# mazpie/genrl

Measured on AMD Instinct MI355X. Metric: world-model+imag update steps/sec (B32xL32x64x64x3), higher is better.
Workload: dtype f32 (storage, accumulation, every non-GEMM kernel and the fp32-MFMA GEMMs; the forward / dgrad / weight-gradient products of the imagination rollout, of the Dense+LN+SiLU chains from 192 rows up and of the encoder / decoder convolutions take fp32 operands pre-split into two fp16 planes of the scaled

## Files before the change

### genrl_amd/csrc/gemm_planes.hip

```cpp
#include "common.h"
#include "genrl_hip.h"
#include <type_traits>

typedef __bf16 bf16x8_t __attribute__((ext_vector_type(8)));
typedef _Float16 f16x8_t __attribute__((ext_vector_type(8)));
typedef unsigned u32x4 __attribute__((ext_vector_type(4)));

namespace {

struct PlaneSeg {
  const u16* a; long a_ld, a_plane;
  const u16* b; long b_ld, b_plane;
  int k;
  const float* a_inv; const float* b_inv;
};

struct SampleEpi {
  const float* q;
  long ldq;
  float* sample; long lds;
  u16* sp; long sld, splane; float* sinv;
  float a;
};

// ... 465 lines not shown
      if (ln.rstd) ln.rstd[row] = rs;
      if (ln.yinv) ln.yinv[row] = u_inv;
    }
    if (row < M) {
#pragma unroll
      for (int gq = 0; gq < 4; ++gq) {
        const int col = n0 + wn * 32 + 8 * gq + 4 * h32;
        const f32x4 g = ldsf4(LN_G + 4 * col), b = ldsf4(LN_B + 4 * col);
        float y[4];
#pragma unroll
        for (int v = 0; v < 4; ++v) {
          const float z = (o[4 * gq + v] - mu) * rs * g[v] + b[v];
          y[v] = ln.act ? siluf_(z) : z;
        }
        if (ln.y) *reinterpret_cast<float4*>(ln.y + (long)row * ln.ldy + col) = make_float4(y[0], y[1], y[2], y[3]);
        if (ln.yp) {
          h2_u32x2 hh, ll;
          unsigned a, bq;
          h2_split2(y[0] * u_sc, y[1] * u_sc, a, bq); hh[0] = a; ll[0] = bq;
          h2_split2(y[2] * u_sc, y[3] * u_sc, a, bq); hh[1] = a; ll[1] = bq;
          u16* qd = ln.yp + (long)row * ln.yld + col;
          *reinterpret_cast<h2_u32x2*>(qd) = hh;
          *reinterpret_cast<h2_u32x2*>(qd + ln.yplane) = ll;
        }
      }
    }
    return;
  }
  const float* ainv = ainv_l;
  const float* binv = binv_l;
  auto epi_f = [&](int idx) __attribute__((always_inline)) -> float {
    return *reinterpret_cast<const __attribute__((address_space(3))) float*>((uintptr_t)(lds0 + EPI_AT + 4 * idx));
  };
  auto epi_f4 = [&](int idx) __attribute__((always_inline)) -> float4 {
    typedef float f32x4_ __attribute__((ext_vector_type(4)));
    const f32x4_ t = *reinterpret_cast<const __attribute__((address_space(3))) f32x4_*>((uintptr_t)(lds0 + EPI_AT + 4 * idx));
    return make_float4(t[0], t[1], t[2], t[3]);
  };
  const bool vec_c = ((ldc & 3) == 0) && (((reinterpret_cast<uintptr_t>(C) | reinterpret_cast<uintptr_t>(bias)) & 15) == 0);
#pragma unroll
  for (int i = 0; i < TM; ++i) {
    const int row = m0 + (wm * TM + i) * 32 + l32;
    if (row >= M) continue;
    const float ra = ainv ? (FMT == 1 ? epi_f((wm * TM + i) * 32 + l32) : ainv[row]) : 1.f;
    float lg[16];
#pragma unroll
    for (int j = 0; j < TN; ++j)
#pragma unroll
      for (int gq = 0; gq < 4; ++gq) {
        const int col = n0 + (wn * TN + j) * 32 + 8 * gq + 4 * h32;
        if (col >= N) continue;
        float o[4];
        float cbv[4] = {1.f, 1.f, 1.f, 1.f}, bsv[4] = {0.f, 0.f, 0.f, 0.f};
        if constexpr (FMT == 1) {
          const int ci = (wn * TN + j) * 32 + 8 * gq + 4 * h32;
          if (binv) { const float4 t = epi_f4(BM + ci); cbv[0] = t.x; cbv[1] = t.y; cbv[2] = t.z; cbv[3] = t.w; }
          if (bias) { const float4 t = epi_f4(BM + BN + ci); bsv[0] = t.x; bsv[1] = t.y; bsv[2] = t.z; bsv[3] = t.w; }
        }
#pragma unroll
        for (int v = 0; v < 4; ++v) {
          if constexpr (FMT == 0) {
            float x = acc[0][i][j][4 * gq + v];
#pragma unroll
            for (int c = 1; c < NACC; ++c) x += acc[c][i][j][4 * gq + v];
            o[v] = x;
          } else {
            const float lo = NACC == 3 ? acc[0][i][j][4 * gq + v] + acc[2][i][j][4 * gq + v] : acc[0][i][j][4 * gq + v];
            const float x = lo * (1.f / 2048.f) + acc[1][i][j][4 * gq + v];
            o[v] = x * ra * cbv[v];
          }
        }
        float* c = C + (long)row * ldc + col;
        if (vec_c && col + 3 < N) {
          if constexpr (FMT == 1) {
            o[0] += bsv[0]; o[1] += bsv[1]; o[2] += bsv[2]; o[3] += bsv[3];
          } else if (bias) {
            const float4 bv = *reinterpret_cast<const float4*>(bias + col);
            o[0] += bv.x; o[1] += bv.y; o[2] += bv.z; o[3] += bv.w;
          }
          if (accumulate) {
            const float4 cv = *reinterpret_cast<const float4*>(c);
            o[0] += cv.x; o[1] += cv.y; o[2] += cv.z; o[3] += cv.w;
          }
          *reinterpret_cast<float4*>(c) = make_float4(o[0], o[1], o[2], o[3]);
          if constexpr (TM * TN == 1 && FMT == 1) {
#pragma unroll
            for (int v = 0; v < 4; ++v) lg[4 * gq + v] = o[v];
          }
        } else {
#pragma unroll
          for (int v = 0; v < 4; ++v)
            if (col + v < N) {
              float val = o[v] + (FMT == 1 ? bsv[v] : (bias ? bias[col + v] : 0.f));
              if (accumulate) val += c[v];
              c[v] = val;
            }
        }
      }
    if constexpr (TM * TN == 1 && FMT == 1) {
      if (smp.q) {
        const int c0 = n0 + wn * 32;
        float m = lg[0];
#pragma unroll
        for (int v = 1; v < 16; ++v) m = fmaxf(m, lg[v]);
        m = fmaxf(m, __shfl_xor(m, 32, 64));
        float e[16], z = 0.f;
#pragma unroll
        for (int v = 0; v < 16; ++v) { e[v] = expf(lg[v] - m); z += e[v]; }
        z += __shfl_xor(z, 32, 64);
        float ssum = 0.f;
#pragma unroll
        for (int v = 0; v < 16; ++v) { e[v] = smp.a * (e[v] / z) + (1.0f - smp.a) / 32.0f; ssum += e[v]; }
        ssum += __shfl_xor(ssum, 32, 64);
        float best = -INFINITY; int bi = 0;
#pragma unroll
        for (int gq = 0; gq < 4; ++gq) {
          const int cl = 8 * gq + 4 * h32;
          const float4 qv = *reinterpret_cast<const float4*>(smp.q + (long)row * smp.ldq + c0 + cl);
          const float qq[4] = {qv.x, qv.y, qv.z, qv.w};
#pragma unroll
          for (int v = 0; v < 4; ++v) {
            const float sc = (e[4 * gq + v] / ssum) / qq[v];
            if (sc > best) { best = sc; bi = cl + v; }
          }
        }
        {
          const float ob = __shfl_xor(best, 32, 64);
          const int oi = __shfl_xor(bi, 32, 64);
          if (ob > best || (ob == best && oi < bi)) { best = ob; bi = oi; }
        }
#pragma unroll
        for (int gq = 0; gq < 4; ++gq) {
          const int cl = 8 * gq + 4 * h32;
          float4 oh;
          oh.x = (cl + 0 == bi) ? 1.f : 0.f; oh.y = (cl + 1 == bi) ? 1.f : 0.f;
          oh.z = (cl + 2 == bi) ? 1.f : 0.f; oh.w = (cl + 3 == bi) ? 1.f : 0.f;
          *reinterpret_cast<float4*>(smp.sample + (long)row * smp.lds + c0 + cl) = oh;
          if (smp.sp) {
            h2_u32x2 hh;
            hh[0] = (oh.x != 0.f ? 0x7400u : 0u) | (oh.y != 0.f ? 0x74000000u : 0u);
            hh[1] = (oh.z != 0.f ? 0x7400u : 0u) | (oh.w != 0.f ? 0x74000000u : 0u);
            u16* qd = smp.sp + (long)row * smp.sld + c0 + cl;
            *reinterpret_cast<h2_u32x2*>(qd) = hh;
            *reinterpret_cast<h2_u32x2*>(qd + smp.splane) = h2_u32x2{0u, 0u};
          }
        }
        if (smp.sinv && c0 == 0 && h32 == 0) smp.sinv[row] = 1.f / 16384.f;
      }
    }
  }
  wait_vm<0>();
}

constexpr int HL_KBH = 2, HL_KBL = 2;
template <bool CONV>
__global__ __launch_bounds__(256, 1) void gemm_planes_hl_kernel(PlaneSeg s0, float* __restrict__ C, long ldc, const float* __restrict__ bias,
                                                                int M, int N, int accumulate, int tiles_m, int tiles_n, int xcd_m,
                                                                ConvGather cg) {
  constexpr int BM = 128, BN = 128, ROWB = 128, HALF = (BM + BN) * ROWB, NS = 4, NP = 8, KS = 4;
  constexpr int EPI = 4 * (BM + 2 * BN), EPI_AT = NS * HALF;
  __shared__ __attribute__((aligned(1024))) unsigned char lds[EPI_AT + EPI];
  int tile_m, tile_n;
  {
    int bid = blockIdx.x;
    const int ntiles = tiles_m * tiles_n;
    const int x = bid % 8, i = bid / 8;
    const int order = xcd_m >> 8;
    xcd_m &= 255;
    if (xcd_m > 0) {
      const int sub_m = tiles_m / xcd_m, sub_n = tiles_n / (8 / xcd_m);
      const int xm = x / (8 / xcd_m), xn = x % (8 / xcd_m);
      int im = i / sub_n, in = i % sub_n;
      if (order == 1 && sub_m % 8 == 0 && sub_n % 4 == 0) {
        const int nb_n = sub_n / 4, blk = i / 32, j = i % 32;
        const int rb = blk / nb_n, cbq = blk % nb_n, cb = (rb & 1) ? nb_n - 1 - cbq : cbq;
        im = rb * 8 + j / 4; in = cb * 4 + j % 4;
      } else if (order == 2) {
        im = i % sub_m; in = i / sub_m;
      }
      tile_m = xm * sub_m + im;
      tile_n = xn * sub_n + in;
    } else {
      const int q = ntiles / 8, r = ntiles % 8;
      bid = (x < r ? x * (q + 1) : r * (q + 1) + (x - r) * q) + i;
      tile_m = bid / tiles_n;
      tile_n = bid % tiles_n;
    }
  }
  const int m0 = tile_m * BM, n0 = tile_n * BN;
  const int lane = threadIdx.x & 63;
  const int wave = __builtin_amdgcn_readfirstlane(threadIdx.x >> 6);
  const int wm = wave >> 1, wn = wave & 1;
  const unsigned lds0 = (unsigned)(uintptr_t)lds;
  const bool isB = wave >= 2;
  const int r_in = lane >> 3, slot = lane & 7;
  const char* gbase = reinterpret_cast<const char*>(isB ? s0.b : s0.a);
  const long plane_bytes = (isB ? s0.b_plane : s0.a_plane) * 2;
  unsigned voff[NP];
  unsigned koff[2] = {0u, 0u};
  int kch[2] = {0, 0}, kkw[2] = {0, 0}, kkk[2] = {0, 0};
  if (CONV && !isB) {
    const long ld = s0.a_ld;
#pragma unroll
    for (int i = 0; i < NP; ++i) {
      const int row = ((wave & 1) * NP + i) * 8 + r_in;
      const int m = min(m0 + row, M - 1);
      const int n_img = m / (cg.Ho * cg.Wo), rem = m - n_img * (cg.Ho * cg.Wo);
      const int oy = rem / cg.Wo, ox = rem - oy * cg.Wo;
      voff[i] = (unsigned)((((long)(n_img * cg.H + cg.s * oy) * cg.W + cg.s * ox) * ld) * 2);
    }
#pragma unroll
    for (int par = 0; par < 2; ++par) {
      const int f = (4 * par + (r_in >> 1)) & 7;
      const int kk = 8 * (slot ^ f);
      const int tap = kk / cg.C, ch = kk - tap * cg.C, kh = tap / cg.k, kw = tap - kh * cg.k;
      kkk[par] = kk; kch[par] = ch; kkw[par] = kw;
      koff[par] = (unsigned)((((long)kh * cg.W + kw) * ld + ch) * 2);
    }
  } else {
    const long ld = isB ? s0.b_ld : s0.a_ld;
    const int rows_total = isB ? N : M, r0 = isB ? n0 : m0;
#pragma unroll
    for (int i = 0; i < NP; ++i) {
      const int row = ((wave & 1) * NP + i) * 8 + r_in;
      const int f = (row >> 1) & 7;
      voff[i] = (unsigned)(((long)min(r0 + row, rows_total - 1) * ld) * 2 + ((slot ^ f) << 4));
    }
  }
  const unsigned piece0 = lds0 + (isB ? BM * ROWB : 0) + (wave & 1) * NP * 1024;
  const int l32 = lane & 31, h32 = lane >> 5;
  const int f_rd = (l32 >> 1) & 7;
  unsigned a_s[KS], b_s[KS];
#pragma unroll
  for (int s = 0; s < KS; ++s) {
    const unsigned xo = (unsigned)(((2 * s + h32) ^ f_rd) << 4);
    a_s[s] = lds0 + (wm * 64 + l32) * ROWB + xo;
    b_s[s] = lds0 + BM * ROWB + (wn * 64 + l32) * ROWB + xo;
  }
  f32x16 acc[2][2][2];
#pragma unroll
  for (int c = 0; c < 2; ++c)
#pragma unroll
    for (int i = 0; i < 2; ++i)
#pragma unroll
      for (int j = 0; j < 2; ++j)
#pragma unroll
        for (int r = 0; r < 16; ++r) acc[c][i][j][r] = 0.f;
  u32x4 Hf[2][KS][4], Lf[KS][4];
  auto ldfrag = [&](unsigned addr) __attribute__((always_inline)) -> u32x4 {
    return *reinterpret_cast<const __attribute__((address_space(3))) u32x4*>((uintptr_t)addr);
  };
  auto read_one = [&](u32x4 (&dst)[KS][4], int r, int buf) __attribute__((always_inline)) {
    const int s = r >> 2, blk = r & 3;
    dst[s][blk] = blk < 2 ? ldfrag(a_s[s] + blk * 32 * ROWB + buf * HALF) : ldfrag(b_s[s] + (blk - 2) * 32 * ROWB + buf * HALF);
  };
  auto mma = [&](f32x16& c, const u32x4& bfr, const u32x4& afr) __attribute__((always_inline)) {
    c = __builtin_amdgcn_mfma_f32_32x32x16_f16(__builtin_bit_cast(f16x8_t, bfr), __builtin_bit_cast(f16x8_t, afr), c, 0, 0, 0);
  };
  {
    const float* src = wave == 0 ? s0.a_inv : (wave == 1 ? s0.b_inv : (wave == 2 ? bias : nullptr));
    const int base = wave == 0 ? m0 : n0, lim = (wave == 0 ? M : N) - 1;
    const unsigned dst = lds0 + EPI_AT + (wave == 0 ? 0 : (wave == 1 ? 4 * BM : 4 * (BM + BN)));
    if (src) {
#pragma unroll
      for (int j = 0; j < 2; ++j)
        __builtin_amdgcn_global_load_lds((const __attribute__((address_space(1))) void*)(src + min(base + 64 * j + lane, lim)),
                                         (__attribute__((address_space(3))) void*)(uintptr_t)(dst + 256 * j), 4, 0, 0);
    }
  }
  const int nu = 2 * (s0.k / 64);
  int issued = 0;
  auto next_half = [&]() __attribute__((always_inline)) {
    if (issued > 0 && issued < nu) {
      if (issued & 1) gbase += plane_bytes;
      else {
        gbase += 128 - plane_bytes;
        if constexpr (CONV) {
          if (!isB) {
            gbase -= 128;
            const unsigned ld2 = (unsigned)(s0.a_ld * 2);
#pragma unroll
            for (int par = 0; par < 2; ++par) {
              if (kkk[par] + 64 + 8 <= cg.K) {
                kkk[par] += 64;
                int ch = kch[par] + 64, kw = kkw[par];
                unsigned off = koff[par] + 128u;
#pragma unroll
                for (int rep = 0; rep < 2; ++rep)
                  if (ch >= cg.C) {
                    ch -= cg.C; off -= (unsigned)(cg.C * 2);
                    ++kw; off += ld2;
                    if (kw == cg.k) { kw = 0; off += (unsigned)(cg.W - cg.k) * ld2; }
                  }
                kch[par] = ch; kkw[par] = kw; koff[par] = off;
              }
            }
          }
        }
      }
    }
    ++issued;
  };
  auto issue_one = [&](int buf, int i) __attribute__((always_inline)) {
    if constexpr (CONV) {
      if (!isB) { glds16(gbase + (size_t)(voff[i] + koff[i & 1]), piece0 + buf * HALF + i * 1024); return; }
    }
    glds16(gbase + (size_t)voff[i], piece0 + buf * HALF + i * 1024);
  };
#pragma unroll
  for (int st = 0; st < NS; ++st) {
    next_half();
#pragma unroll
    for (int i = 0; i < NP; ++i) issue_one(st, i);
  }
  next_half();
  wait_vm<(NS - 1) * NP>();
  __builtin_amdgcn_s_barrier();
#pragma unroll
  for (int r = 0; r < 16; ++r) read_one(Hf[0], r, 0);

  int u = 0;
  auto half_iter = [&](auto UC) __attribute__((always_inline)) {
    constexpr int U = decltype(UC)::value;
    constexpr bool LPH = (U & 1) != 0;
    constexpr int HS = U >> 1;
    constexpr int NM = LPH ? 32 : 16, KB = LPH ? HL_KBL : HL_KBH, NSIDE = 16 + NP;
    constexpr int PER = (NSIDE + (NM - KB) - 1) / (NM - KB);
    static_assert((NSIDE + PER - 1) / PER <= NM - KB, "not enough MFMAs to carry the side operations");
    auto mfma_one = [&](int m) __attribute__((always_inline)) {
      if constexpr (!LPH) {
        const int s = m >> 2, i = (m >> 1) & 1, j = m & 1;
        mma(acc[1][i][j], Hf[HS][s][2 + j], Hf[HS][s][i]);
      } else {
        const int s = m >> 3, t = (m >> 2) & 1, i = (m >> 1) & 1, j = m & 1;
        if (t == 0) mma(acc[0][i][j], Hf[HS][s][2 + j], Lf[s][i]);
        else mma(acc[0][i][j], Lf[s][2 + j], Hf[HS][s][i]);
      }
    };
#pragma unroll
    for (int m = 0; m < KB; ++m) mfma_one(m);
    __builtin_amdgcn_sched_barrier(0);
    wait_vm<(NS - 2) * NP>();
    asm volatile("s_waitcnt lgkmcnt(0)" ::: "memory");
    __builtin_amdgcn_s_barrier();
    __builtin_amdgcn_sched_barrier(0);
#pragma unroll
    for (int m = KB; m < NM; ++m) {
      mfma_one(m);
#pragma unroll
      for (int o = (m - KB) * PER; o < (m - KB + 1) * PER; ++o) {
        if (o >= NSIDE) continue;
        if (o % 3 == 2) {
          issue_one(U, o / 3);
        } else {
          const int r = o - o / 3;
          if constexpr (LPH) read_one(Hf[1 - HS], r, (U + 1) % NS);
          else read_one(Lf, r, (U + 1) % NS);
        }
      }
      __builtin_amdgcn_sched_barrier(0);
    }
    next_half();
    ++u;
  };
  while (u + 4 <= nu) {
    half_iter(std::integral_constant<int, 0>{});
    half_iter(std::integral_constant<int, 1>{});
    half_iter(std::integral_constant<int, 2>{});
    half_iter(std::integral_constant<int, 3>{});
  }
  if (u < nu) {
    half_iter(std::integral_constant<int, 0>{});
    half_iter(std::integral_constant<int, 1>{});
  }

  auto epi_f = [&](int idx) __attribute__((always_inline)) -> float {
    return *reinterpret_cast<const __attribute__((address_space(3))) float*>((uintptr_t)(lds0 + EPI_AT + 4 * idx));
  };
  auto epi_f4 = [&](int idx) __attribute__((always_inline)) -> float4 {
    typedef float f32x4_ __attribute__((ext_vector_type(4)));
    const f32x4_ t = *reinterpret_cast<const __attribute__((address_space(3))) f32x4_*>((uintptr_t)(lds0 + EPI_AT + 4 * idx));
    return make_float4(t[0], t[1], t[2], t[3]);
  };
  const bool vec_c = ((ldc & 3) == 0) && (((reinterpret_cast<uintptr_t>(C) | reinterpret_cast<uintptr_t>(bias)) & 15) == 0);
  const bool shuffle = CONV && cg.sCo > 0;
#pragma unroll
  for (int i = 0; i < 2; ++i) {
    const int row = m0 + (wm * 2 + i) * 32 + l32;
    if (row >= M) continue;
    const float ra = s0.a_inv ? epi_f((wm * 2 + i) * 32 + l32) : 1.f;
    int s_py = 0, s_px = 0; long s_img = 0;
    if (shuffle) {
      const int per = cg.Ho * cg.Wo, n_img = row / per, rem = row - n_img * per;
      s_py = rem / cg.Wo; s_px = rem - s_py * cg.Wo;
      s_img = (long)n_img * cg.sHo;
    }
#pragma unroll
    for (int j = 0; j < 2; ++j)
#pragma unroll
      for (int gq = 0; gq < 4; ++gq) {
        const int ci = (wn * 2 + j) * 32 + 8 * gq + 4 * h32, col = n0 + ci;
        if (col >= N) continue;
        float cbv[4] = {1.f, 1.f, 1.f, 1.f}, bsv[4] = {0.f, 0.f, 0.f, 0.f};
        if (s0.b_inv) { const float4 t = epi_f4(BM + ci); cbv[0] = t.x; cbv[1] = t.y; cbv[2] = t.z; cbv[3] = t.w; }
        if (bias) { const float4 t = epi_f4(BM + BN + ci); bsv[0] = t.x; bsv[1] = t.y; bsv[2] = t.z; bsv[3] = t.w; }
        float o[4];
#pragma unroll
        for (int v = 0; v < 4; ++v)
          o[v] = (acc[0][i][j][4 * gq + v] * (1.f / 2048.f) + acc[1][i][j][4 * gq + v]) * ra * cbv[v] + bsv[v];
        if (shuffle) {
          const int cls = col / cg.sCo, co = col - cls * cg.sCo;
          const int oy = 2 * s_py + (cls >> 1), ox = 2 * s_px + (cls & 1);
          if (oy < cg.sHo && ox < cg.sWo)
            *reinterpret_cast<float4*>(C + ((s_img + oy) * cg.sWo + ox) * cg.sCo + co) = make_float4(o[0], o[1], o[2], o[3]);
          continue;
        }
        float* c = C + (long)row * ldc + col;
        if (vec_c && col + 3 < N) {
          if (accumulate) {
            const float4 cv = *reinterpret_cast<const float4*>(c);
            o[0] += cv.x; o[1] += cv.y; o[2] += cv.z; o[3] += cv.w;
          }
          *reinterpret_cast<float4*>(c) = make_float4(o[0], o[1], o[2], o[3]);
        } else {
#pragma unroll
          for (int v = 0; v < 4; ++v)
            if (col + v < N) c[v] = accumulate ? c[v] + o[v] : o[v];
        }
      }
  }
  wait_vm<0>();
}

template <bool CONV, int TJ, int WGM = 2>
__global__ __launch_bounds__(256, 1) void gemm_planes_hlw_kernel(PlaneSeg s0, float* __restrict__ C, long ldc, const float* __restrict__ bias,
                                                                 int M, int N, int accumulate, int tiles_m, int tiles_n, int xcd_m,
                                                                 ConvGather cg) {
  constexpr int WGN = 4 / WGM, BM = 64 * WGM, BN = 32 * TJ * WGN, ROWB = 128, HALF = (BM + BN) * ROWB, NS = 3, KS = 4, NB = 2 + TJ;
  constexpr int APIECES = BM / 8, NPT = (BM + BN) / 8, NP = NPT / 4;
  static_assert(NPT % 4 == 0, "pieces deal evenly over four waves");
  constexpr int EPI = 4 * (BM + 2 * BN), EPI_AT = NS * HALF;
  __shared__ __attribute__((aligned(1024))) unsigned char lds[EPI_AT + EPI];
  int tile_m, tile_n;
  {
    int bid = blockIdx.x;
    const int ntiles = tiles_m * tiles_n;
    const int x = bid % 8, i = bid / 8;
    if (xcd_m > 0) {
      const int sub_m = tiles_m / xcd_m, sub_n = tiles_n / (8 / xcd_m);
      const int xm = x / (8 / xcd_m), xn = x % (8 / xcd_m);
      tile_m = xm * sub_m + i / sub_n;
      tile_n = xn * sub_n + i % sub_n;
    } else {
      const int q = ntiles / 8, r = ntiles % 8;
      bid = (x < r ? x * (q + 1) : r * (q + 1) + (x - r) * q) + i;
      tile_m = bid / tiles_n;
      tile_n = bid % tiles_n;
    }
  }
  const int m0 = tile_m * BM, n0 = tile_n * BN;
  const int lane = threadIdx.x & 63;
  const int wave = __builtin_amdgcn_readfirstlane(threadIdx.x >> 6);
  const int wm = WGM == 2 ? (wave >> 1) : wave, wn = WGM == 2 ? (wave & 1) : 0;
  const unsigned lds0 = (unsigned)(uintptr_t)lds;
  const int r_in = lane >> 3, slot = lane & 7;
  const char* gA = reinterpret_cast<const char*>(s0.a);
  const char* gB = reinterpret_cast<const char*>(s0.b);
  const long pbA = s0.a_plane * 2, pbB = s0.b_plane * 2;
  unsigned voff[NP];
  unsigned koff[2] = {0u, 0u};
  int kch[2] = {0, 0}, kkw[2] = {0, 0}, kkk[2] = {0, 0};
#pragma unroll
  for (int i = 0; i < NP; ++i) {
    const int p = wave * NP + i;
    if (p < APIECES) {
      const int row = p * 8 + r_in;
      if constexpr (CONV) {
        const int m = min(m0 + row, M - 1);
        const int n_img = m / (cg.Ho * cg.Wo), rem = m - n_img * (cg.Ho * cg.Wo);
        const int oy = rem / cg.Wo, ox = rem - oy * cg.Wo;
        voff[i] = (unsigned)((((long)(n_img * cg.H + cg.s * oy) * cg.W + cg.s * ox) * s0.a_ld) * 2);
      } else {
        voff[i] = (unsigned)(((long)min(m0 + row, M - 1) * s0.a_ld) * 2 + ((slot ^ ((row >> 1) & 7)) << 4));
      }
    } else {
      const int row = (p - APIECES) * 8 + r_in;
      voff[i] = (unsigned)(((long)min(n0 + row, N - 1) * s0.b_ld) * 2 + ((slot ^ ((row >> 1) & 7)) << 4));
    }
  }
  if constexpr (CONV) {
#pragma unroll
    for (int par = 0; par < 2; ++par) {
      const int f = (4 * par + (r_in >> 1)) & 7;
      const int kk = 8 * (slot ^ f);
      const int tap = kk / cg.C, ch = kk - tap * cg.C, kh = tap / cg.k, kw = tap - kh * cg.k;
      kkk[par] = kk; kch[par] = ch; kkw[par] = kw;
      koff[par] = (unsigned)((((long)kh * cg.W + kw) * s0.a_ld + ch) * 2);
    }
  }
  const unsigned piece0 = lds0 + wave * NP * 1024;
  const int l32 = lane & 31, h32 = lane >> 5;
  const int f_rd = (l32 >> 1) & 7;
  unsigned a_s[KS], b_s[KS];
#pragma unroll
  for (int s = 0; s < KS; ++s) {
    const unsigned xo = (unsigned)(((2 * s + h32) ^ f_rd) << 4);
    a_s[s] = lds0 + (wm * 64 + l32) * ROWB + xo;
    b_s[s] = lds0 + BM * ROWB + (wn * 32 * TJ + l32) * ROWB + xo;
  }
  f32x16 acc[2][2][TJ];
#pragma unroll
  for (int c = 0; c < 2; ++c)
#pragma unroll
    for (int i = 0; i < 2; ++i)
#pragma unroll
      for (int j = 0; j < TJ; ++j)
#pragma unroll
        for (int r = 0; r < 16; ++r) acc[c][i][j][r] = 0.f;
  u32x4 Hf[2][KS][NB], Lf[KS][NB];
  auto ldfrag = [&](unsigned addr) __attribute__((always_inline)) -> u32x4 {
    return *reinterpret_cast<const __attribute__((address_space(3))) u32x4*>((uintptr_t)addr);
  };
  auto read_one = [&](u32x4 (&dst)[KS][NB], int r, int buf) __attribute__((always_inline)) {
    const int s = r / NB, blk = r % NB;
    dst[s][blk] = blk < 2 ? ldfrag(a_s[s] + blk * 32 * ROWB + buf * HALF) : ldfrag(b_s[s] + (blk - 2) * 32 * ROWB + buf * HALF);
  };
  auto mma = [&](f32x16& c, const u32x4& bfr, const u32x4& afr) __attribute__((always_inline)) {
    c = __builtin_amdgcn_mfma_f32_32x32x16_f16(__builtin_bit_cast(f16x8_t, bfr), __builtin_bit_cast(f16x8_t, afr), c, 0, 0, 0);
  };
  {
    const float* src = wave == 0 ? s0.a_inv : (wave == 1 ? s0.b_inv : (wave == 2 ? bias : nullptr));
    const int base = wave == 0 ? m0 : n0, lim = (wave == 0 ? M : N) - 1;
    const unsigned dst = lds0 + EPI_AT + (wave == 0 ? 0 : (wave == 1 ? 4 * BM : 4 * (BM + BN)));
    if (src) {
#pragma unroll
      for (int j = 0; j < ((BM > BN ? BM : BN) + 63) / 64; ++j)
        if (64 * j + lane < (wave == 0 ? BM : BN))
          __builtin_amdgcn_global_load_lds((const __attribute__((address_space(1))) void*)(src + min(base + 64 * j + lane, lim)),
                                           (__attribute__((address_space(3))) void*)(uintptr_t)(dst + 256 * j), 4, 0, 0);
    }
  }
  const int nu = 2 * (s0.k / 64);
  int issued = 0;
  auto next_half = [&]() __attribute__((always_inline)) {
    if (issued > 0 && issued < nu) {
      if (issued & 1) { gA += pbA; gB += pbB; }
      else {
        gB += 128 - pbB;
        if constexpr (CONV) {
          gA -= pbA;
          const unsigned ld2 = (unsigned)(s0.a_ld * 2);
#pragma unroll
          for (int par = 0; par < 2; ++par) {
            if (kkk[par] + 64 + 8 <= cg.K) {
              kkk[par] += 64;
              int ch = kch[par] + 64, kw = kkw[par];
              unsigned off = koff[par] + 128u;
#pragma unroll
              for (int rep = 0; rep < 2; ++rep)
                if (ch >= cg.C) {
                  ch -= cg.C; off -= (unsigned)(cg.C * 2);
                  ++kw; off += ld2;
                  if (kw == cg.k) { kw = 0; off += (unsigned)(cg.W - cg.k) * ld2; }
                }
              kch[par] = ch; kkw[par] = kw; koff[par] = off;
            }
          }
        } else {
          gA += 128 - pbA;
        }
      }
    }
    ++issued;
  };
  auto issue_one = [&](int buf, int i) __attribute__((always_inline)) {
    const int p = wave * NP + i;
    const unsigned dst = piece0 + buf * HALF + i * 1024;
    if (p < APIECES) {
      if constexpr (CONV) glds16(gA + (size_t)(voff[i] + koff[p & 1]), dst);
      else glds16(gA + (size_t)voff[i], dst);
    } else {
      glds16(gB + (size_t)voff[i], dst);
    }
  };
#pragma unroll
  for (int st = 0; st < NS; ++st) {
    next_half();
#pragma unroll
    for (int i = 0; i < NP; ++i) issue_one(st, i);
  }
  next_half();
  wait_vm<(NS - 1) * NP>();
  __builtin_amdgcn_s_barrier();
#pragma unroll
  for (int r = 0; r < KS * NB; ++r) read_one(Hf[0], r, 0);

  int u = 0;
  auto half_iter = [&](auto BC, auto LC, auto HC) __attribute__((always_inline)) {
    constexpr int BUF = decltype(BC)::value, HS = decltype(HC)::value;
    constexpr bool LPH = decltype(LC)::value != 0;
    constexpr int NM = LPH ? 4 * KS * TJ : 2 * KS * TJ, KB = 2, NSIDE = KS * NB + NP;
    constexpr int PER = (NSIDE + (NM - KB) - 1) / (NM - KB);
    static_assert((NSIDE + PER - 1) / PER <= NM - KB, "not enough MFMAs to carry the side operations");
    constexpr int NR = KS * NB, NPAIR = NP < NR / 2 ? NP : NR / 2;
    auto mfma_one = [&](int m) __attribute__((always_inline)) {
      if constexpr (!LPH) {
        const int s = m / (2 * TJ), i = (m / TJ) % 2, j = m % TJ;
        mma(acc[1][i][j], Hf[HS][s][2 + j], Hf[HS][s][i]);
      } else {
        const int s = m / (4 * TJ), t = (m / (2 * TJ)) % 2, i = (m / TJ) % 2, j = m % TJ;
        if (t == 0) mma(acc[0][i][j], Hf[HS][s][2 + j], Lf[s][i]);
        else mma(acc[0][i][j], Lf[s][2 + j], Hf[HS][s][i]);
      }
    };
#pragma unroll
    for (int m = 0; m < KB; ++m) mfma_one(m);
    __builtin_amdgcn_sched_barrier(0);
    wait_vm<(NS - 2) * NP>();
    asm volatile("s_waitcnt lgkmcnt(0)" ::: "memory");
    __builtin_amdgcn_s_barrier();
    __builtin_amdgcn_sched_barrier(0);
#pragma unroll
    for (int m = KB; m < NM; ++m) {
      mfma_one(m);
#pragma unroll
      for (int o = (m - KB) * PER; o < (m - KB + 1) * PER; ++o) {
        if (o >= NSIDE) continue;
        const bool tri = o < 3 * NPAIR;
        const bool dma = tri ? (o % 3 == 2) : (NR == 2 * NPAIR);
        if (dma) {
          issue_one(BUF, tri ? o / 3 : NPAIR + (o - 3 * NPAIR));
        } else {
          const int r = tri ? o - o / 3 : 2 * NPAIR + (o - 3 * NPAIR);
          if constexpr (LPH) read_one(Hf[1 - HS], r, (BUF + 1) % NS);
          else read_one(Lf, r, (BUF + 1) % NS);
        }
      }
      __builtin_amdgcn_sched_barrier(0);
    }
    next_half();
    ++u;
  };
  using I0 = std::integral_constant<int, 0>; using I1 = std::integral_constant<int, 1>; using I2 = std::integral_constant<int, 2>;
#define HLW_PAIR(B0, B1, H) half_iter(B0{}, I0{}, H{}); half_iter(B1{}, I1{}, H{})
  while (u + 12 <= nu) {
    HLW_PAIR(I0, I1, I0); HLW_PAIR(I2, I0, I1); HLW_PAIR(I1, I2, I0); HLW_PAIR(I0, I1, I1); HLW_PAIR(I2, I0, I0); HLW_PAIR(I1, I2, I1);
  }
  if (u + 2 <= nu) { HLW_PAIR(I0, I1, I0); }
  if (u + 2 <= nu) { HLW_PAIR(I2, I0, I1); }
  if (u + 2 <= nu) { HLW_PAIR(I1, I2, I0); }
  if (u + 2 <= nu) { HLW_PAIR(I0, I1, I1); }
  if (u + 2 <= nu) { HLW_PAIR(I2, I0, I0); }
#undef HLW_PAIR

  auto epi_f = [&](int idx) __attribute__((always_inline)) -> float {
    return *reinterpret_cast<const __attribute__((address_space(3))) float*>((uintptr_t)(lds0 + EPI_AT + 4 * idx));
  };
  auto epi_f4 = [&](int idx) __attribute__((always_inline)) -> float4 {
    typedef float f32x4_ __attribute__((ext_vector_type(4)));
    const f32x4_ t = *reinterpret_cast<const __attribute__((address_space(3))) f32x4_*>((uintptr_t)(lds0 + EPI_AT + 4 * idx));
    return make_float4(t[0], t[1], t[2], t[3]);
  };
  const bool vec_c = ((ldc & 3) == 0) && (((reinterpret_cast<uintptr_t>(C) | reinterpret_cast<uintptr_t>(bias)) & 15) == 0);
  const bool shuffle = CONV && cg.sCo > 0;
#pragma unroll
  for (int i = 0; i < 2; ++i) {
    const int row = m0 + (wm * 2 + i) * 32 + l32;
    if (row >= M) continue;
    const float ra = s0.a_inv ? epi_f((wm * 2 + i) * 32 + l32) : 1.f;
    int s_py = 0, s_px = 0; long s_img = 0;
    if (shuffle) {
      const int per = cg.Ho * cg.Wo, n_img = row / per, rem = row - n_img * per;
      s_py = rem / cg.Wo; s_px = rem - s_py * cg.Wo;
      s_img = (long)n_img * cg.sHo;
    }
#pragma unroll
    for (int j = 0; j < TJ; ++j)
#pragma unroll
      for (int gq = 0; gq < 4; ++gq) {
        const int ci = (wn * TJ + j) * 32 + 8 * gq + 4 * h32, col = n0 + ci;
        if (col >= N) continue;
        float cbv[4] = {1.f, 1.f, 1.f, 1.f}, bsv[4] = {0.f, 0.f, 0.f, 0.f};
        if (s0.b_inv) { const float4 t = epi_f4(BM + ci); cbv[0] = t.x; cbv[1] = t.y; cbv[2] = t.z; cbv[3] = t.w; }
        if (bias) { const float4 t = epi_f4(BM + BN + ci); bsv[0] = t.x; bsv[1] = t.y; bsv[2] = t.z; bsv[3] = t.w; }
        float o[4];
#pragma unroll
        for (int v = 0; v < 4; ++v)
          o[v] = (acc[0][i][j][4 * gq + v] * (1.f / 2048.f) + acc[1][i][j][4 * gq + v]) * ra * cbv[v] + bsv[v];
        if (shuffle) {
          const int cls = col / cg.sCo, co = col - cls * cg.sCo;
          const int oy = 2 * s_py + (cls >> 1), ox = 2 * s_px + (cls & 1);
          if (oy < cg.sHo && ox < cg.sWo)
            *reinterpret_cast<float4*>(C + ((s_img + oy) * cg.sWo + ox) * cg.sCo + co) = make_float4(o[0], o[1], o[2], o[3]);
          continue;
        }
        float* c = C + (long)row * ldc + col;
        if (vec_c && col + 3 < N) {
          if (accumulate) {
            const float4 cv = *reinterpret_cast<const float4*>(c);
            o[0] += cv.x; o[1] += cv.y; o[2] += cv.z; o[3] += cv.w;
          }
          *reinterpret_cast<float4*>(c) = make_float4(o[0], o[1], o[2], o[3]);
        } else {
#pragma unroll
          for (int v = 0; v < 4; ++v)
            if (col + v < N) c[v] = accumulate ? c[v] + o[v] : o[v];
        }
      }
  }
  wait_vm<0>();
}

__device__ __forceinline__ unsigned bf16_rne(float x) {
  const unsigned u = __builtin_bit_cast(unsigned, x);
  return (u + 0x7FFFu + ((u >> 16) & 1u)) >> 16;
}
__device__ __forceinline__ void split3(float x, u16& h, u16& m, u16& l) {
  const unsigned uh = bf16_rne(x);
  const float r1 = x - __builtin_bit_cast(float, uh << 16);
  const unsigned um = bf16_rne(r1);
  const float r2 = r1 - __builtin_bit_cast(float, um << 16);
  h = (u16)uh; m = (u16)um; l = (u16)bf16_rne(r2);
}

__global__ __launch_bounds__(256) void split_x3_kernel(const float* __restrict__ x, long ldx, int R, int Cn,
                                                       u16* __restrict__ out, long ld_out, long plane, int transpose) {
  __shared__ float tile[32][33];
  const int tx = threadIdx.x & 31, ty = threadIdx.x >> 5;
  const int ro = blockIdx.y * 32, co = blockIdx.x * 32;
  const int Ro = transpose ? Cn : R, Co = transpose ? R : Cn;
#pragma unroll
  for (int k = 0; k < 4; ++k) {
    const int a = ty + 8 * k;
    float v = 0.f;
    if (!transpose) {
      const int r = ro + a, c = co + tx;
      if (r < R && c < Cn) v = x[(long)r * ldx + c];
      tile[a][tx] = v;
    } else {
      const int r = co + a, c = ro + tx;
      if (r < R && c < Cn) v = x[(long)r * ldx + c];
      tile[tx][a] = v;
    }
  }
  __syncthreads();
#pragma unroll
  for (int k = 0; k < 4; ++k) {
    const int a = ty + 8 * k;
    const int r = ro + a, c = co + tx;
    if (r < Ro && c < ld_out) {
      u16 h, m, l;
      split3(c < Co ? tile[a][tx] : 0.f, h, m, l);
      u16* o = out + (long)r * ld_out + c;
      o[0] = h; o[plane] = m; o[2 * plane] = l;
    }
  }
}

__global__ __launch_bounds__(256) void split_h2_rows_kernel(const float* __restrict__ x, long ldx, int R, int Cn,
                                                            u16* __restrict__ out, long ld_out, long plane,
                                                            float* __restrict__ inv) {
  const int row = blockIdx.x * 4 + (threadIdx.x >> 6), lane = threadIdx.x & 63;
  if (row >= R) return;
  const float* xr = x + (long)row * ldx;
  float m = 0.f;
  for (int c = lane; c < Cn; c += 64) m = fmaxf(m, fabsf(xr[c]));
  const float iv = h2_inv_of(wave_max(m)), sc = h2_scale_of(iv);
  if (lane == 0) inv[row] = iv;
  u16* o = out + (long)row * ld_out;
  for (int c = 2 * lane; c < ld_out; c += 128) {
    unsigned h, l;
    h2_split2(c < Cn ? xr[c] * sc : 0.f, c + 1 < Cn ? xr[c + 1] * sc : 0.f, h, l);
    *reinterpret_cast<unsigned*>(o + c) = h;
    *reinterpret_cast<unsigned*>(o + plane + c) = l;
  }
}

__global__ __launch_bounds__(256) void h2_colmax_kernel(const float* __restrict__ x, long ldx, int R, int Cn,
                                                        float* __restrict__ inv) {
  __shared__ float part[8][32];
  const int tx = threadIdx.x & 31, ty = threadIdx.x >> 5;
  const int c = blockIdx.x * 32 + tx;
  float m = 0.f;
  if (c < Cn) {
    int r = ty;
    for (; r + 56 < R; r += 64) {
      float v[8];
#pragma unroll
      for (int u = 0; u < 8; ++u) v[u] = x[(long)(r + 8 * u) * ldx + c];
#pragma unroll
      for (int u = 0; u < 8; ++u) m = fmaxf(m, fabsf(v[u]));
    }
    for (; r < R; r += 8) m = fmaxf(m, fabsf(x[(long)r * ldx + c]));
  }
  part[ty][tx] = m;
  __syncthreads();
  if (ty == 0 && c < Cn) {
#pragma unroll
    for (int k = 1; k < 8; ++k) m = fmaxf(m, part[k][tx]);
    inv[c] = h2_inv_of(m);
  }
}

__global__ __launch_bounds__(256) void split_h2_t_kernel(const float* __restrict__ x, long ldx, int R, int Cn,
                                                         u16* __restrict__ out, long ld_out, long plane,
                                                         const float* __restrict__ inv) {
  __shared__ float tile[32][33];
  const int tx = threadIdx.x & 31, ty = threadIdx.x >> 5;
  const int ro = blockIdx.y * 32, co = blockIdx.x * 32;
#pragma unroll
  for (int k = 0; k < 4; ++k) {
    const int a = ty + 8 * k;
    const int r = co + a, c = ro + tx;
    tile[tx][a] = (r < R && c < Cn) ? x[(long)r * ldx + c] : 0.f;
  }
  __syncthreads();
#pragma unroll
  for (int k = 0; k < 4; ++k) {
    const int a = ty + 8 * k;
    const int r = ro + a, c = co + tx;
    if (r < Cn && c < ld_out) {
      unsigned h, l;
      h2_split2(c < R ? tile[a][tx] * h2_scale_of(inv[r]) : 0.f, 0.f, h, l);
      u16* o = out + (long)r * ld_out + c;
      o[0] = (u16)(h & 0xFFFFu); o[plane] = (u16)(l & 0xFFFFu);
    }
  }
}

struct SplitEntry {
  const float* src; long ldx; int R, Cn;
  u16* out; long ld_out, plane; float* inv;
};
struct SplitBatch {
  int n;
  int blk0[33];
  SplitEntry e[32];
};
__device__ __forceinline__ int batch_entry(const SplitBatch& b, int blk) {
  int i = 0;
  while (i + 1 < b.n && blk >= b.blk0[i + 1]) ++i;
  return i;
}
__global__ __launch_bounds__(256) void split_h2_rows_batch_kernel(SplitBatch b) {
  const int i = batch_entry(b, blockIdx.x);
  const SplitEntry& e = b.e[i];
  const int row = (blockIdx.x - b.blk0[i]) * 4 + (threadIdx.x >> 6), lane = threadIdx.x & 63;
  if (row >= e.R) return;
  const float* xr = e.src + (long)row * e.ldx;
  float m = 0.f;
  for (int c = lane; c < e.Cn; c += 64) m = fmaxf(m, fabsf(xr[c]));
  const float iv = h2_inv_of(wave_max(m)), sc = h2_scale_of(iv);
  if (lane == 0) e.inv[row] = iv;
  u16* o = e.out + (long)row * e.ld_out;
  for (int c = 2 * lane; c < e.ld_out; c += 128) {
    unsigned h, l;
    h2_split2(c < e.Cn ? xr[c] * sc : 0.f, c + 1 < e.Cn ? xr[c + 1] * sc : 0.f, h, l);
    *reinterpret_cast<unsigned*>(o + c) = h;
    *reinterpret_cast<unsigned*>(o + e.plane + c) = l;
  }
}
// ... 369 lines not shown
```

Baseline: 45.52.

## Switch split-plane GEMM kernels from 32x32x16 to 16x16x32 fp16 MFMA tiles

```diff
diff --git a/genrl_amd/csrc/gemm_planes.hip b/genrl_amd/csrc/gemm_planes.hip
--- a/genrl_amd/csrc/gemm_planes.hip
+++ b/genrl_amd/csrc/gemm_planes.hip
@@ -641,12 +641,13 @@
   wait_vm<0>();
 }
 
+__device__ __forceinline__ void hl_mfma_drain() { asm volatile("s_nop 15\n\ts_nop 15" ::: "memory"); }
 constexpr int HL_KBH = 2, HL_KBL = 2;
 template <bool CONV>
 __global__ __launch_bounds__(256, 1) void gemm_planes_hl_kernel(PlaneSeg s0, float* __restrict__ C, long ldc, const float* __restrict__ bias,
                                                                 int M, int N, int accumulate, int tiles_m, int tiles_n, int xcd_m,
                                                                 ConvGather cg) {
-  constexpr int BM = 128, BN = 128, ROWB = 128, HALF = (BM + BN) * ROWB, NS = 4, NP = 8, KS = 4;
+  constexpr int BM = 128, BN = 128, ROWB = 128, HALF = (BM + BN) * ROWB, NS = 4, NP = 8, KS = 2;
   constexpr int EPI = 4 * (BM + 2 * BN), EPI_AT = NS * HALF;
   __shared__ __attribute__((aligned(1024))) unsigned char lds[EPI_AT + EPI];
   int tile_m, tile_n;
@@ -717,34 +718,34 @@
     }
   }
   const unsigned piece0 = lds0 + (isB ? BM * ROWB : 0) + (wave & 1) * NP * 1024;
-  const int l32 = lane & 31, h32 = lane >> 5;
-  const int f_rd = (l32 >> 1) & 7;
+  const int l16 = lane & 15, q16 = lane >> 4;
+  const int f_rd = (l16 >> 1) & 7;
   unsigned a_s[KS], b_s[KS];
 #pragma unroll
   for (int s = 0; s < KS; ++s) {
-    const unsigned xo = (unsigned)(((2 * s + h32) ^ f_rd) << 4);
-    a_s[s] = lds0 + (wm * 64 + l32) * ROWB + xo;
-    b_s[s] = lds0 + BM * ROWB + (wn * 64 + l32) * ROWB + xo;
-  }
-  f32x16 acc[2][2][2];
+    const unsigned xo = (unsigned)(((4 * s + q16) ^ f_rd) << 4);
+    a_s[s] = lds0 + (wm * 64 + l16) * ROWB + xo;
+    b_s[s] = lds0 + BM * ROWB + (wn * 64 + l16) * ROWB + xo;
+  }
+  f32x4 acc[2][4][4];
 #pragma unroll
   for (int c = 0; c < 2; ++c)
 #pragma unroll
-    for (int i = 0; i < 2; ++i)
-#pragma unroll
-      for (int j = 0; j < 2; ++j)
-#pragma unroll
-        for (int r = 0; r < 16; ++r) acc[c][i][j][r] = 0.f;
-  u32x4 Hf[2][KS][4], Lf[KS][4];
+    for (int i = 0; i < 4; ++i)
+#pragma unroll
+      for (int j = 0; j < 4; ++j)
+#pragma unroll
+        for (int r = 0; r < 4; ++r) acc[c][i][j][r] = 0.f;
+  u32x4 Hf[2][KS][8], Lf[KS][8];
   auto ldfrag = [&](unsigned addr) __attribute__((always_inline)) -> u32x4 {
     return *reinterpret_cast<const __attribute__((address_space(3))) u32x4*>((uintptr_t)addr);
   };
-  auto read_one = [&](u32x4 (&dst)[KS][4], int r, int buf) __attribute__((always_inline)) {
-    const int s = r >> 2, blk = r & 3;
-    dst[s][blk] = blk < 2 ? ldfrag(a_s[s] + blk * 32 * ROWB + buf * HALF) : ldfrag(b_s[s] + (blk - 2) * 32 * ROWB + buf * HALF);
-  };
-  auto mma = [&](f32x16& c, const u32x4& bfr, const u32x4& afr) __attribute__((always_inline)) {
-    c = __builtin_amdgcn_mfma_f32_32x32x16_f16(__builtin_bit_cast(f16x8_t, bfr), __builtin_bit_cast(f16x8_t, afr), c, 0, 0, 0);
+  auto read_one = [&](u32x4 (&dst)[KS][8], int r, int buf) __attribute__((always_inline)) {
+    const int s = r >> 3, blk = r & 7;
+    dst[s][blk] = blk < 4 ? ldfrag(a_s[s] + blk * 16 * ROWB + buf * HALF) : ldfrag(b_s[s] + (blk - 4) * 16 * ROWB + buf * HALF);
+  };
+  auto mma = [&](f32x4& c, const u32x4& bfr, const u32x4& afr) __attribute__((always_inline)) {
+    asm volatile("v_mfma_f32_16x16x32_f16 %0, %1, %2, %0" : "+a"(c) : "v"(bfr), "v"(afr));
   };
   {
     const float* src = wave == 0 ? s0.a_inv : (wave == 1 ? s0.b_inv : (wave == 2 ? bias : nullptr));
@@ -813,17 +814,17 @@
     constexpr int U = decltype(UC)::value;
     constexpr bool LPH = (U & 1) != 0;
     constexpr int HS = U >> 1;
-    constexpr int NM = LPH ? 32 : 16, KB = LPH ? HL_KBL : HL_KBH, NSIDE = 16 + NP;
+    constexpr int NM = LPH ? 64 : 32, KB = LPH ? HL_KBL : HL_KBH, NSIDE = 16 + NP;
     constexpr int PER = (NSIDE + (NM - KB) - 1) / (NM - KB);
     static_assert((NSIDE + PER - 1) / PER <= NM - KB, "not enough MFMAs to carry the side operations");
     auto mfma_one = [&](int m) __attribute__((always_inline)) {
       if constexpr (!LPH) {
-        const int s = m >> 2, i = (m >> 1) & 1, j = m & 1;
-        mma(acc[1][i][j], Hf[HS][s][2 + j], Hf[HS][s][i]);
+        const int s = m >> 4, i = (m >> 2) & 3, j = m & 3;
+        mma(acc[1][i][j], Hf[HS][s][4 + j], Hf[HS][s][i]);
       } else {
-        const int s = m >> 3, t = (m >> 2) & 1, i = (m >> 1) & 1, j = m & 1;
-        if (t == 0) mma(acc[0][i][j], Hf[HS][s][2 + j], Lf[s][i]);
-        else mma(acc[0][i][j], Lf[s][2 + j], Hf[HS][s][i]);
+        const int s = m >> 5, t = (m >> 4) & 1, i = (m >> 2) & 3, j = m & 3;
+        if (t == 0) mma(acc[0][i][j], Hf[HS][s][4 + j], Lf[s][i]);
+        else mma(acc[0][i][j], Lf[s][4 + j], Hf[HS][s][i]);
       }
     };
 #pragma unroll
@@ -863,6 +864,7 @@
     half_iter(std::integral_constant<int, 1>{});
   }
 
+  hl_mfma_drain();
   auto epi_f = [&](int idx) __attribute__((always_inline)) -> float {
     return *reinterpret_cast<const __attribute__((address_space(3))) float*>((uintptr_t)(lds0 + EPI_AT + 4 * idx));
   };
@@ -874,10 +876,10 @@
   const bool vec_c = ((ldc & 3) == 0) && (((reinterpret_cast<uintptr_t>(C) | reinterpret_cast<uintptr_t>(bias)) & 15) == 0);
   const bool shuffle = CONV && cg.sCo > 0;
 #pragma unroll
-  for (int i = 0; i < 2; ++i) {
-    const int row = m0 + (wm * 2 + i) * 32 + l32;
+  for (int i = 0; i < 4; ++i) {
+    const int row = m0 + (wm * 4 + i) * 16 + l16;
     if (row >= M) continue;
-    const float ra = s0.a_inv ? epi_f((wm * 2 + i) * 32 + l32) : 1.f;
+    const float ra = s0.a_inv ? epi_f((wm * 4 + i) * 16 + l16) : 1.f;
     int s_py = 0, s_px = 0; long s_img = 0;
     if (shuffle) {
       const int per = cg.Ho * cg.Wo, n_img = row / per, rem = row - n_img * per;
@@ -885,38 +887,36 @@
       s_img = (long)n_img * cg.sHo;
     }
 #pragma unroll
-    for (int j = 0; j < 2; ++j)
-#pragma unroll
-      for (int gq = 0; gq < 4; ++gq) {
-        const int ci = (wn * 2 + j) * 32 + 8 * gq + 4 * h32, col = n0 + ci;
-        if (col >= N) continue;
-        float cbv[4] = {1.f, 1.f, 1.f, 1.f}, bsv[4] = {0.f, 0.f, 0.f, 0.f};
-        if (s0.b_inv) { const float4 t = epi_f4(BM + ci); cbv[0] = t.x; cbv[1] = t.y; cbv[2] = t.z; cbv[3] = t.w; }
-        if (bias) { const float4 t = epi_f4(BM + BN + ci); bsv[0] = t.x; bsv[1] = t.y; bsv[2] = t.z; bsv[3] = t.w; }
-        float o[4];
+    for (int j = 0; j < 4; ++j) {
+      const int ci = (wn * 4 + j) * 16 + 4 * q16, col = n0 + ci;
+      if (col >= N) continue;
+      float cbv[4] = {1.f, 1.f, 1.f, 1.f}, bsv[4] = {0.f, 0.f, 0.f, 0.f};
+      if (s0.b_inv) { const float4 t = epi_f4(BM + ci); cbv[0] = t.x; cbv[1] = t.y; cbv[2] = t.z; cbv[3] = t.w; }
+      if (bias) { const float4 t = epi_f4(BM + BN + ci); bsv[0] = t.x; bsv[1] = t.y; bsv[2] = t.z; bsv[3] = t.w; }
+      float o[4];
+#pragma unroll
+      for (int v = 0; v < 4; ++v)
+        o[v] = (acc[0][i][j][v] * (1.f / 2048.f) + acc[1][i][j][v]) * ra * cbv[v] + bsv[v];
+      if (shuffle) {
+        const int cls = col / cg.sCo, co = col - cls * cg.sCo;
+        const int oy = 2 * s_py + (cls >> 1), ox = 2 * s_px + (cls & 1);
+        if (oy < cg.sHo && ox < cg.sWo)
+          *reinterpret_cast<float4*>(C + ((s_img + oy) * cg.sWo + ox) * cg.sCo + co) = make_float4(o[0], o[1], o[2], o[3]);
+        continue;
+      }
+      float* c = C + (long)row * ldc + col;
+      if (vec_c && col + 3 < N) {
+        if (accumulate) {
+          const float4 cv = *reinterpret_cast<const float4*>(c);
+          o[0] += cv.x; o[1] += cv.y; o[2] += cv.z; o[3] += cv.w;
+        }
+        *reinterpret_cast<float4*>(c) = make_float4(o[0], o[1], o[2], o[3]);
+      } else {
 #pragma unroll
         for (int v = 0; v < 4; ++v)
-          o[v] = (acc[0][i][j][4 * gq + v] * (1.f / 2048.f) + acc[1][i][j][4 * gq + v]) * ra * cbv[v] + bsv[v];
-        if (shuffle) {
-          const int cls = col / cg.sCo, co = col - cls * cg.sCo;
-          const int oy = 2 * s_py + (cls >> 1), ox = 2 * s_px + (cls & 1);
-          if (oy < cg.sHo && ox < cg.sWo)
-            *reinterpret_cast<float4*>(C + ((s_img + oy) * cg.sWo + ox) * cg.sCo + co) = make_float4(o[0], o[1], o[2], o[3]);
-          continue;
-        }
-        float* c = C + (long)row * ldc + col;
-        if (vec_c && col + 3 < N) {
-          if (accumulate) {
-            const float4 cv = *reinterpret_cast<const float4*>(c);
-            o[0] += cv.x; o[1] += cv.y; o[2] += cv.z; o[3] += cv.w;
-          }
-          *reinterpret_cast<float4*>(c) = make_float4(o[0], o[1], o[2], o[3]);
-        } else {
-#pragma unroll
-          for (int v = 0; v < 4; ++v)
-            if (col + v < N) c[v] = accumulate ? c[v] + o[v] : o[v];
-        }
-      }
+          if (col + v < N) c[v] = accumulate ? c[v] + o[v] : o[v];
+      }
+    }
   }
   wait_vm<0>();
 }
@@ -925,7 +925,7 @@
 __global__ __launch_bounds__(256, 1) void gemm_planes_hlw_kernel(PlaneSeg s0, float* __restrict__ C, long ldc, const float* __restrict__ bias,
                                                                  int M, int N, int accumulate, int tiles_m, int tiles_n, int xcd_m,
                                                                  ConvGather cg) {
-  constexpr int WGN = 4 / WGM, BM = 64 * WGM, BN = 32 * TJ * WGN, ROWB = 128, HALF = (BM + BN) * ROWB, NS = 3, KS = 4, NB = 2 + TJ;
+  constexpr int WGN = 4 / WGM, BM = 64 * WGM, BN = 32 * TJ * WGN, ROWB = 128, HALF = (BM + BN) * ROWB, NS = 3, KS = 2, NJ = 2 * TJ, NB = 4 + NJ;
   constexpr int APIECES = BM / 8, NPT = (BM + BN) / 8, NP = NPT / 4;
   static_assert(NPT % 4 == 0, "pieces deal evenly over four waves");
   constexpr int EPI = 4 * (BM + 2 * BN), EPI_AT = NS * HALF;
@@ -988,34 +988,34 @@
     }
   }
   const unsigned piece0 = lds0 + wave * NP * 1024;
-  const int l32 = lane & 31, h32 = lane >> 5;
-  const int f_rd = (l32 >> 1) & 7;
+  const int l16 = lane & 15, q16 = lane >> 4;
+  const int f_rd = (l16 >> 1) & 7;
   unsigned a_s[KS], b_s[KS];
 #pragma unroll
   for (int s = 0; s < KS; ++s) {
-    const unsigned xo = (unsigned)(((2 * s + h32) ^ f_rd) << 4);
-    a_s[s] = lds0 + (wm * 64 + l32) * ROWB + xo;
-    b_s[s] = lds0 + BM * ROWB + (wn * 32 * TJ + l32) * ROWB + xo;
-  }
-  f32x16 acc[2][2][TJ];
+    const unsigned xo = (unsigned)(((4 * s + q16) ^ f_rd) << 4);
+    a_s[s] = lds0 + (wm * 64 + l16) * ROWB + xo;
+    b_s[s] = lds0 + BM * ROWB + (wn * 32 * TJ + l16) * ROWB + xo;
+  }
+  f32x4 acc[2][4][NJ];
 #pragma unroll
   for (int c = 0; c < 2; ++c)
 #pragma unroll
-    for (int i = 0; i < 2; ++i)
-#pragma unroll
-      for (int j = 0; j < TJ; ++j)
-#pragma unroll
-        for (int r = 0; r < 16; ++r) acc[c][i][j][r] = 0.f;
+    for (int i = 0; i < 4; ++i)
+#pragma unroll
+      for (int j = 0; j < NJ; ++j)
+#pragma unroll
+        for (int r = 0; r < 4; ++r) acc[c][i][j][r] = 0.f;
   u32x4 Hf[2][KS][NB], Lf[KS][NB];
   auto ldfrag = [&](unsigned addr) __attribute__((always_inline)) -> u32x4 {
     return *reinterpret_cast<const __attribute__((address_space(3))) u32x4*>((uintptr_t)addr);
   };
   auto read_one = [&](u32x4 (&dst)[KS][NB], int r, int buf) __attribute__((always_inline)) {
     const int s = r / NB, blk = r % NB;
-    dst[s][blk] = blk < 2 ? ldfrag(a_s[s] + blk * 32 * ROWB + buf * HALF) : ldfrag(b_s[s] + (blk - 2) * 32 * ROWB + buf * HALF);
-  };
-  auto mma = [&](f32x16& c, const u32x4& bfr, const u32x4& afr) __attribute__((always_inline)) {
-    c = __builtin_amdgcn_mfma_f32_32x32x16_f16(__builtin_bit_cast(f16x8_t, bfr), __builtin_bit_cast(f16x8_t, afr), c, 0, 0, 0);
+    dst[s][blk] = blk < 4 ? ldfrag(a_s[s] + blk * 16 * ROWB + buf * HALF) : ldfrag(b_s[s] + (blk - 4) * 16 * ROWB + buf * HALF);
+  };
+  auto mma = [&](f32x4& c, const u32x4& bfr, const u32x4& afr) __attribute__((always_inline)) {
+    asm volatile("v_mfma_f32_16x16x32_f16 %0, %1, %2, %0" : "+a"(c) : "v"(bfr), "v"(afr));
   };
   {
     const float* src = wave == 0 ? s0.a_inv : (wave == 1 ? s0.b_inv : (wave == 2 ? bias : nullptr));
@@ -1088,18 +1088,18 @@
   auto half_iter = [&](auto BC, auto LC, auto HC) __attribute__((always_inline)) {
     constexpr int BUF = decltype(BC)::value, HS = decltype(HC)::value;
     constexpr bool LPH = decltype(LC)::value != 0;
-    constexpr int NM = LPH ? 4 * KS * TJ : 2 * KS * TJ, KB = 2, NSIDE = KS * NB + NP;
+    constexpr int NM = (LPH ? 8 : 4) * KS * NJ, KB = 2, NSIDE = KS * NB + NP;
     constexpr int PER = (NSIDE + (NM - KB) - 1) / (NM - KB);
     static_assert((NSIDE + PER - 1) / PER <= NM - KB, "not enough MFMAs to carry the side operations");
     constexpr int NR = KS * NB, NPAIR = NP < NR / 2 ? NP : NR / 2;
     auto mfma_one = [&](int m) __attribute__((always_inline)) {
       if constexpr (!LPH) {
-        const int s = m / (2 * TJ), i = (m / TJ) % 2, j = m % TJ;
-        mma(acc[1][i][j], Hf[HS][s][2 + j], Hf[HS][s][i]);
+        const int s = m / (4 * NJ), i = (m / NJ) % 4, j = m % NJ;
+        mma(acc[1][i][j], Hf[HS][s][4 + j], Hf[HS][s][i]);
       } else {
-        const int s = m / (4 * TJ), t = (m / (2 * TJ)) % 2, i = (m / TJ) % 2, j = m % TJ;
-        if (t == 0) mma(acc[0][i][j], Hf[HS][s][2 + j], Lf[s][i]);
-        else mma(acc[0][i][j], Lf[s][2 + j], Hf[HS][s][i]);
+        const int s = m / (8 * NJ), t = (m / (4 * NJ)) % 2, i = (m / NJ) % 4, j = m % NJ;
+        if (t == 0) mma(acc[0][i][j], Hf[HS][s][4 + j], Lf[s][i]);
+        else mma(acc[0][i][j], Lf[s][4 + j], Hf[HS][s][i]);
       }
     };
 #pragma unroll
@@ -1142,6 +1142,7 @@
   if (u + 2 <= nu) { HLW_PAIR(I2, I0, I0); }
 #undef HLW_PAIR
 
+  hl_mfma_drain();
   auto epi_f = [&](int idx) __attribute__((always_inline)) -> float {
     return *reinterpret_cast<const __attribute__((address_space(3))) float*>((uintptr_t)(lds0 + EPI_AT + 4 * idx));
   };
@@ -1153,10 +1154,10 @@
   const bool vec_c = ((ldc & 3) == 0) && (((reinterpret_cast<uintptr_t>(C) | reinterpret_cast<uintptr_t>(bias)) & 15) == 0);
   const bool shuffle = CONV && cg.sCo > 0;
 #pragma unroll
-  for (int i = 0; i < 2; ++i) {
-    const int row = m0 + (wm * 2 + i) * 32 + l32;
+  for (int i = 0; i < 4; ++i) {
+    const int row = m0 + (wm * 4 + i) * 16 + l16;
     if (row >= M) continue;
-    const float ra = s0.a_inv ? epi_f((wm * 2 + i) * 32 + l32) : 1.f;
+    const float ra = s0.a_inv ? epi_f((wm * 4 + i) * 16 + l16) : 1.f;
     int s_py = 0, s_px = 0; long s_img = 0;
     if (shuffle) {
       const int per = cg.Ho * cg.Wo, n_img = row / per, rem = row - n_img * per;
@@ -1164,38 +1165,36 @@
       s_img = (long)n_img * cg.sHo;
     }
 #pragma unroll
-    for (int j = 0; j < TJ; ++j)
-#pragma unroll
-      for (int gq = 0; gq < 4; ++gq) {
-        const int ci = (wn * TJ + j) * 32 + 8 * gq + 4 * h32, col = n0 + ci;
-        if (col >= N) continue;
-        float cbv[4] = {1.f, 1.f, 1.f, 1.f}, bsv[4] = {0.f, 0.f, 0.f, 0.f};
-        if (s0.b_inv) { const float4 t = epi_f4(BM + ci); cbv[0] = t.x; cbv[1] = t.y; cbv[2] = t.z; cbv[3] = t.w; }
-        if (bias) { const float4 t = epi_f4(BM + BN + ci); bsv[0] = t.x; bsv[1] = t.y; bsv[2] = t.z; bsv[3] = t.w; }
-        float o[4];
+    for (int j = 0; j < NJ; ++j) {
+      const int ci = (wn * NJ + j) * 16 + 4 * q16, col = n0 + ci;
+      if (col >= N) continue;
+      float cbv[4] = {1.f, 1.f, 1.f, 1.f}, bsv[4] = {0.f, 0.f, 0.f, 0.f};
+      if (s0.b_inv) { const float4 t = epi_f4(BM + ci); cbv[0] = t.x; cbv[1] = t.y; cbv[2] = t.z; cbv[3] = t.w; }
+      if (bias) { const float4 t = epi_f4(BM + BN + ci); bsv[0] = t.x; bsv[1] = t.y; bsv[2] = t.z; bsv[3] = t.w; }
+      float o[4];
+#pragma unroll
+      for (int v = 0; v < 4; ++v)
+        o[v] = (acc[0][i][j][v] * (1.f / 2048.f) + acc[1][i][j][v]) * ra * cbv[v] + bsv[v];
+      if (shuffle) {
+        const int cls = col / cg.sCo, co = col - cls * cg.sCo;
+        const int oy = 2 * s_py + (cls >> 1), ox = 2 * s_px + (cls & 1);
+        if (oy < cg.sHo && ox < cg.sWo)
+          *reinterpret_cast<float4*>(C + ((s_img + oy) * cg.sWo + ox) * cg.sCo + co) = make_float4(o[0], o[1], o[2], o[3]);
+        continue;
+      }
+      float* c = C + (long)row * ldc + col;
+      if (vec_c && col + 3 < N) {
+        if (accumulate) {
+          const float4 cv = *reinterpret_cast<const float4*>(c);
+          o[0] += cv.x; o[1] += cv.y; o[2] += cv.z; o[3] += cv.w;
+        }
+        *reinterpret_cast<float4*>(c) = make_float4(o[0], o[1], o[2], o[3]);
+      } else {
 #pragma unroll
         for (int v = 0; v < 4; ++v)
-          o[v] = (acc[0][i][j][4 * gq + v] * (1.f / 2048.f) + acc[1][i][j][4 * gq + v]) * ra * cbv[v] + bsv[v];
-        if (shuffle) {
-          const int cls = col / cg.sCo, co = col - cls * cg.sCo;
-          const int oy = 2 * s_py + (cls >> 1), ox = 2 * s_px + (cls & 1);
-          if (oy < cg.sHo && ox < cg.sWo)
-            *reinterpret_cast<float4*>(C + ((s_img + oy) * cg.sWo + ox) * cg.sCo + co) = make_float4(o[0], o[1], o[2], o[3]);
-          continue;
-        }
-        float* c = C + (long)row * ldc + col;
-        if (vec_c && col + 3 < N) {
-          if (accumulate) {
-            const float4 cv = *reinterpret_cast<const float4*>(c);
-            o[0] += cv.x; o[1] += cv.y; o[2] += cv.z; o[3] += cv.w;
-          }
-          *reinterpret_cast<float4*>(c) = make_float4(o[0], o[1], o[2], o[3]);
-        } else {
-#pragma unroll
-          for (int v = 0; v < 4; ++v)
-            if (col + v < N) c[v] = accumulate ? c[v] + o[v] : o[v];
-        }
-      }
+          if (col + v < N) c[v] = accumulate ? c[v] + o[v] : o[v];
+      }
+    }
   }
   wait_vm<0>();
 }
```

Result: no change. 45.69 (median of 6 runs) (+0.4%).
